# PrimeIntellect-ai/prime

Measured on AMD Instinct MI355X. Metric: tokens_per_sec, higher is better.
Workload: dtype bf16; 1 GPU; model=intellect_10b, global_batch=8, seq_len=2048, parallelism=diloco1_h100_int8ring

## Files before the change

### prime_amd/ops/_lib.py

```python
from __future__ import annotations

import ctypes
from typing import Optional

import torch

from .build import LIB_PATH, build, needs_build

_LIB: Optional[ctypes.CDLL] = None
_TRIED = False

_SIGS = {
    "prime_rmsnorm_fwd": [ctypes.c_void_p] * 5 + [ctypes.c_int64] * 2 + [ctypes.c_double],
    "prime_rmsnorm_bwd": [ctypes.c_void_p] * 7 + [ctypes.c_int64] * 3 + [ctypes.c_double],
    "prime_add_rmsnorm_fwd": [ctypes.c_void_p] * 7 + [ctypes.c_int64] * 2 + [ctypes.c_double],
    "prime_add_rmsnorm_bwd": [ctypes.c_void_p] * 8 + [ctypes.c_int64] * 3 + [ctypes.c_double],
    "prime_rope": [ctypes.c_void_p] * 5 + [ctypes.c_int64] * 4 + [ctypes.c_int, ctypes.c_int64, ctypes.c_void_p],
    "prime_rope_strided": [ctypes.c_void_p] * 5 + [ctypes.c_int64] * 7,
    "prime_qkv_grad_pack": [ctypes.c_void_p] * 8 + [ctypes.c_int64] * 6,
    "prime_swiglu_bwd_t": [ctypes.c_void_p] * 5 + [ctypes.c_int64] * 2,
    "prime_swiglu_fwd": [ctypes.c_void_p] * 3 + [ctypes.c_int64] * 2,
    "prime_swiglu_bwd": [ctypes.c_void_p] * 4 + [ctypes.c_int64] * 2,
    "prime_adamw": [ctypes.c_void_p] * 7 + [ctypes.c_int64] + [ctypes.c_double] * 5 + [ctypes.c_int64],
    "prime_grad_sqnorm": [ctypes.c_void_p] * 3 + [ctypes.c_int64] * 2,
    "prime_grad_sqnorm_partials": [],
    "prime_pseudograd": [ctypes.c_void_p] * 4 + [ctypes.c_int64],
    "prime_quant_int8": [ctypes.c_void_p] * 4 + [ctypes.c_int64],
    "prime_dequant_int8": [ctypes.c_void_p] * 4 + [ctypes.c_int64] * 2,
    "prime_nesterov_outer": [ctypes.c_void_p] * 6 + [ctypes.c_int64] + [ctypes.c_double] * 2,
    "prime_cross_entropy": [ctypes.c_void_p] * 5 + [ctypes.c_int64] * 2 + [ctypes.c_double] + [ctypes.c_int64] * 2,
    "prime_flash_fwd": [ctypes.c_void_p] * 6 + [ctypes.c_int64] * 5 + [ctypes.c_double] + [ctypes.c_int64] * 7 + [ctypes.c_void_p],
    "prime_attn_delta": [ctypes.c_void_p] * 4 + [ctypes.c_int64] * 2,
    "prime_flash_bwd_dq": [ctypes.c_void_p] * 9 + [ctypes.c_int64] * 5 + [ctypes.c_double] + [ctypes.c_int64] * 10 + [ctypes.c_void_p],
    "prime_flash_bwd_dkv": [ctypes.c_void_p] * 13 + [ctypes.c_int64] * 6 + [ctypes.c_double] + [ctypes.c_int64] * 10 + [ctypes.c_void_p],
    "prime_mfma_probe": [ctypes.c_void_p] * 4,
    "prime_mfma_probe32": [ctypes.c_void_p] * 4,
    "prime_transpose_bshd": [ctypes.c_void_p] * 3 + [ctypes.c_int64] * 7,
    "prime_attn_decode": [ctypes.c_void_p] * 5 + [ctypes.c_int64] * 6 + [ctypes.c_double, ctypes.c_void_p],
    "prime_attn_decode_ragged": [ctypes.c_void_p] * 7 + [ctypes.c_int64] * 6 + [ctypes.c_double],
    "prime_decode_ragged_chunk": [],
    "prime_decode_qkv_append": [ctypes.c_void_p] * 8 + [ctypes.c_int64] * 6,
    "prime_gemm_nt": [ctypes.c_void_p] * 4 + [ctypes.c_int64] * 4,
    "prime_gemm_nt8": [ctypes.c_void_p] * 4 + [ctypes.c_int64] * 4,
    "prime_quant_fp8": [ctypes.c_void_p] * 6 + [ctypes.c_int64] * 2,
    "prime_rowwise_quant_fp8": [ctypes.c_void_p] * 4 + [ctypes.c_int64] * 3,
    "prime_transpose_fp8": [ctypes.c_void_p] * 3 + [ctypes.c_int64] * 7 + [ctypes.c_void_p] * 3 + [ctypes.c_int64],
}


def _load() -> ctypes.CDLL:
    import os

    override = os.environ.get("PRIME_AMD_LIB_PATH")
    path = override or str(LIB_PATH)
    if override is None and needs_build():
        build(verbose=True)
    lib = ctypes.CDLL(path)
    for name, argtypes in _SIGS.items():
        try:
            fn = getattr(lib, name)
        except AttributeError:
            continue
        fn.argtypes = argtypes
        fn.restype = ctypes.c_int
    return lib


def lib() -> ctypes.CDLL:
    global _LIB, _TRIED
    if _LIB is None:
        if _TRIED:
            raise RuntimeError("prime_amd HIP kernel library failed to load earlier")
        _TRIED = True
        try:
            _LIB = _load()
        except Exception as e:
            raise RuntimeError(
                "prime_amd requires its HIP kernel library on GPU machines; "
                f"build failed or .so missing at {LIB_PATH}: {e}"
            ) from e
    return _LIB


def have_lib() -> bool:
    try:
        lib()
        return True
    except RuntimeError:
        return False


def stream_of(t: torch.Tensor) -> ctypes.c_void_p:
    s = torch.cuda.current_stream(t.device).cuda_stream
    return ctypes.c_void_p(s)


def check(ret: int, what: str) -> None:
    if ret != 0:
        raise RuntimeError(f"HIP kernel {what} failed with hipError_t={ret}")


def ptr(t: Optional[torch.Tensor]) -> ctypes.c_void_p:
    if t is None:
        return ctypes.c_void_p(0)
    return ctypes.c_void_p(t.data_ptr())
```

### prime_amd/ops/csrc/attention.hip

```cpp
#include "common.h"
#include <stdlib.h>

typedef __attribute__((ext_vector_type(8))) short short8;
typedef __attribute__((ext_vector_type(4))) float f32x4;
typedef __attribute__((address_space(3))) char lds_char;
typedef __attribute__((address_space(3))) void lds_void;
typedef __attribute__((address_space(1))) const void g_void;

__device__ __forceinline__ short8 ld8(const bf16* p) {
  return *reinterpret_cast<const short8*>(p);
}

__device__ __forceinline__ f32x4 mfma16(short8 a, short8 b, f32x4 c) {
  return __builtin_amdgcn_mfma_f32_16x16x32_bf16(a, b, c, 0, 0, 0);
}

__device__ __forceinline__ float grp16_max(float x) {
#pragma unroll
  for (int off = 1; off < 16; off <<= 1) x = fmaxf(x, __shfl_xor(x, off, 64));
  return x;
}
__device__ __forceinline__ float grp16_sum(float x) {
#pragma unroll
  for (int off = 1; off < 16; off <<= 1) x += __shfl_xor(x, off, 64);
// ... 610 lines not shown

  const bf16* Qb = Q + b * sqb + h * sqh;
  const bf16* Kb = K + b * skb + hkv * skh;
  const bf16* Vb = V + b * svb + hkv * svh;
  const bf16* Ktb = Kt + ((int64_t)(b * Hkv + hkv) * D) * S;
  const bf16* dOb = dO + ((int64_t)b * S * H + h) * D;
  const float* lse_b = lse + (int64_t)b * S * H + h;
  const float* dl_b = delta + (int64_t)b * S * H + h;

  __shared__ bf16 k_lds[64 * D];
  __shared__ bf16 v_lds[64 * D];
  __shared__ bf16 kt_lds[D * 64];
  __shared__ bf16 ds_lds_all[4][16 * 64];
  bf16* ds_lds = ds_lds_all[wid];

  short8 qf[DS], dof[DS];
#pragma unroll
  for (int ds = 0; ds < DS; ++ds) {
    qf[ds] = ld8(Qb + (int64_t)(q0 + li) * sqs + ds * 32 + lg * 8);
    dof[ds] = ld8(dOb + (int64_t)(q0 + li) * H * D + ds * 32 + lg * 8);
  }
  float lse_r[4], dl_r[4];
#pragma unroll
  for (int r = 0; r < 4; ++r) {
    lse_r[r] = lse_b[(int64_t)(q0 + lg * 4 + r) * H];
    dl_r[r] = dl_b[(int64_t)(q0 + lg * 4 + r) * H];
  }
  f32x4 dq_acc[DT];
#pragma unroll
  for (int dt = 0; dt < DT; ++dt) dq_acc[dt] = f32x4{0.f, 0.f, 0.f, 0.f};

  const int kv_end = causal ? (qt * 64 + 64) : S;
  int kv_begin = 0, my_kv_begin = 0, row_ds[4];
  if (DOC) {
    const int* doc_b = doc + (int64_t)b * S;
    kv_begin = doc_clamp(doc_b[qt * 64], qt * 64) & ~63;
    my_kv_begin = doc_clamp(doc_b[q0], q0) & ~63;
#pragma unroll
    for (int r = 0; r < 4; ++r) row_ds[r] = doc_b[q0 + lg * 4 + r];
  }
  for (int kv = kv_begin; kv < kv_end; kv += 64) {
    __syncthreads();
    stage_tile<64, D>(Kb + (int64_t)kv * sks, sks, k_lds, threadIdx.x);
    stage_tile<64, D>(Vb + (int64_t)kv * svs, svs, v_lds, threadIdx.x);
    stage_tile<D, 64>(Ktb + kv, S, kt_lds, threadIdx.x);
    __syncthreads();
    if (DOC && kv < my_kv_begin) continue;
#pragma unroll
    for (int sub = 0; sub < 4; ++sub) {
      f32x4 s_acc{0.f, 0.f, 0.f, 0.f}, dp_acc{0.f, 0.f, 0.f, 0.f};
#pragma unroll
      for (int ds = 0; ds < DS; ++ds) {
        s_acc = mfma16(qf[ds], ld8_swz<D>(k_lds, sub * 16 + li, ds * 64 + lg * 16), s_acc);
        dp_acc = mfma16(dof[ds], ld8_swz<D>(v_lds, sub * 16 + li, ds * 64 + lg * 16), dp_acc);
      }
#pragma unroll
      for (int r = 0; r < 4; ++r) {
        const int qg = q0 + lg * 4 + r;
        const int kg = kv + sub * 16 + li;
        float p = __expf(s_acc[r] * scale - lse_r[r]);
        if (causal && kg > qg) p = 0.f;
        if (DOC && kg < row_ds[r]) p = 0.f;
        st16_swz<64>(ds_lds, lg * 4 + r, sub * 16 + li,
                     f2bf(p * (dp_acc[r] - dl_r[r]) * scale));
      }
    }
    wave_lds_fence();
#pragma unroll
    for (int dt = 0; dt < DT; ++dt)
#pragma unroll
      for (int ks = 0; ks < 2; ++ks)
        dq_acc[dt] = mfma16(ld8_swz<64>(ds_lds, li, ks * 64 + lg * 16),
                            ld8_swz<64>(kt_lds, dt * 16 + li, ks * 64 + lg * 16),
                            dq_acc[dt]);
  }
#pragma unroll
  for (int r = 0; r < 4; ++r) {
    bf16* row = dQ + (((int64_t)(b * S + q0 + lg * 4 + r)) * H + h) * D;
#pragma unroll
    for (int dt = 0; dt < DT; ++dt) row[dt * 16 + li] = f2bf(dq_acc[dt][r]);
  }
}

template <int D, int FLAGS>
__global__ __launch_bounds__(512, 2) void flash_bwd_dkv_v5_kernel(
    const bf16* __restrict__ Q, const bf16* __restrict__ Qt,
    const bf16* __restrict__ K, const bf16* __restrict__ V,
    const bf16* __restrict__ dO, const bf16* __restrict__ dOt,
    const float* __restrict__ lse, const float* __restrict__ delta,
    float* __restrict__ wsK, float* __restrict__ wsV, int B, int H, int Hkv,
    int S, float scale, int causal, int splits,
    int64_t sqb, int64_t sqs, int64_t sqh,
    int64_t skb, int64_t sks, int64_t skh,
    int64_t svb, int64_t svs, int64_t svh) {
  constexpr int DSL = D / 16;
  constexpr int DT32 = D / 32;
  const int n_kt = S / 256;
  const int per_split = (B * Hkv) * n_kt;
  const int split = blockIdx.x / per_split;
  const int rem = blockIdx.x - split * per_split;
  const int bh = rem / n_kt;
  const int kt = rem - bh * n_kt;
  const int b = bh / Hkv, hkv = bh - b * Hkv;
  const int group = H / Hkv;
  const int wid = threadIdx.x >> 6;
  const int lane = threadIdx.x & 63;
  const int lo = lane & 31, hi = lane >> 5;
  const int k0w = kt * 256 + wid * 32;

  const bf16* Kb = K + b * skb + hkv * skh;
  const bf16* Vb = V + b * svb + hkv * svh;

  __shared__ bf16 q_lds[2][64 * D];
  __shared__ bf16 do_lds[2][64 * D];
  __shared__ bf16 qt_lds[2][D * 64];
  __shared__ bf16 dot_lds[2][D * 64];

  const bf16* krow = Kb + (int64_t)(k0w + lo) * sks;
  const bf16* vrow = Vb + (int64_t)(k0w + lo) * svs;
  f32x16 dk_acc[DT32], dv_acc[DT32];
#pragma unroll
  for (int dt = 0; dt < DT32; ++dt)
#pragma unroll
    for (int r = 0; r < 16; ++r) { dk_acc[dt][r] = 0.f; dv_acc[dt][r] = 0.f; }

  const int q_start = (causal ? kt * 256 : 0) + split * 64;
  const int tiles_per_g = (S - q_start + 64 * splits - 1) / (64 * splits);
  const int n_iter = group * tiles_per_g;
  const auto stage_for = [&](int it, int buf) {
    const int g = it / tiles_per_g;
    const int q0g = q_start + (it - g * tiles_per_g) * 64 * splits;
    const int h = hkv * group + g;
    const bf16* Qb_ = Q + b * sqb + h * sqh;
    const bf16* dOb_ = dO + ((int64_t)b * S * H + h) * D;
    const bf16* Qtb = Qt + ((int64_t)(b * H + h) * D) * S;
    const bf16* dOtb = dOt + ((int64_t)(b * H + h) * D) * S;
    stage_tile<64, D, 512>(Qb_ + (int64_t)q0g * sqs, sqs, q_lds[buf], threadIdx.x);
    stage_tile<64, D, 512>(dOb_ + (int64_t)q0g * H * D, (int64_t)H * D, do_lds[buf], threadIdx.x);
    stage_tile<D, 64, 512>(Qtb + q0g, S, qt_lds[buf], threadIdx.x);
    stage_tile<D, 64, 512>(dOtb + q0g, S, dot_lds[buf], threadIdx.x);
  };
  stage_for(0, 0);
  for (int it = 0; it < n_iter; ++it) {
    const int cur = it & 1;
    __syncthreads();
    if (it + 1 < n_iter)
      stage_for(it + 1, cur ^ 1);
    const int g = it / tiles_per_g;
    const int q0g = q_start + (it - g * tiles_per_g) * 64 * splits;
    if (causal && q0g + 64 <= k0w) continue;
    const int h = hkv * group + g;
    const float* lse_b = lse + (int64_t)b * S * H + h;
    const float* dl_b = delta + (int64_t)b * S * H + h;

#pragma unroll
    for (int qs = 0; qs < 2; ++qs) {
      const int q32 = q0g + qs * 32;
      f32x16 st, dpt;
#pragma unroll
      for (int r = 0; r < 16; ++r) { st[r] = 0.f; dpt[r] = 0.f; }
      if (FLAGS & 1) __builtin_amdgcn_s_setprio(1);
#pragma unroll
      for (int ds = 0; ds < DSL; ++ds) {
        const short8 qfr = ld8_swz<D>(q_lds[cur], qs * 32 + lo, ds * 32 + hi * 16);
        st = mfma32(qfr, ld8(krow + ds * 16 + hi * 8), st);
      }
#pragma unroll
      for (int ds = 0; ds < DSL; ++ds) {
        const short8 dofr = ld8_swz<D>(do_lds[cur], qs * 32 + lo, ds * 32 + hi * 16);
        dpt = mfma32(dofr, ld8(vrow + ds * 16 + hi * 8), dpt);
      }
      if (FLAGS & 1) __builtin_amdgcn_s_setprio(0);
#pragma unroll
      for (int r = 0; r < 16; ++r) {
        const int qg = q32 + (r & 3) + 8 * (r >> 2) + 4 * hi;
        const float lse_q = lse_b[(int64_t)qg * H];
        const float dl_q = dl_b[(int64_t)qg * H];
        float p = __expf(st[r] * scale - lse_q);
        if (causal && (k0w + lo) > qg) p = 0.f;
        st[r] = p;
        dpt[r] = p * (dpt[r] - dl_q) * scale;
      }
      short8 pa[2], da[2];
#pragma unroll
      for (int kst = 0; kst < 2; ++kst) {
        const int g0 = 4 * (2 * kst), g1 = 4 * (2 * kst + 1);
        unsigned x0 = cvt_pk_bf16(st[g0 + 0], st[g0 + 1]);
        unsigned x1 = cvt_pk_bf16(st[g0 + 2], st[g0 + 3]);
        unsigned y0 = cvt_pk_bf16(st[g1 + 0], st[g1 + 1]);
        unsigned y1 = cvt_pk_bf16(st[g1 + 2], st[g1 + 3]);
        permlane32_swap(x0, y0);
        permlane32_swap(x1, y1);
        short8 f;
        reinterpret_cast<unsigned*>(&f)[0] = x0;
        reinterpret_cast<unsigned*>(&f)[1] = x1;
        reinterpret_cast<unsigned*>(&f)[2] = y0;
        reinterpret_cast<unsigned*>(&f)[3] = y1;
        pa[kst] = f;
        x0 = cvt_pk_bf16(dpt[g0 + 0], dpt[g0 + 1]);
        x1 = cvt_pk_bf16(dpt[g0 + 2], dpt[g0 + 3]);
        y0 = cvt_pk_bf16(dpt[g1 + 0], dpt[g1 + 1]);
        y1 = cvt_pk_bf16(dpt[g1 + 2], dpt[g1 + 3]);
        permlane32_swap(x0, y0);
        permlane32_swap(x1, y1);
        reinterpret_cast<unsigned*>(&f)[0] = x0;
        reinterpret_cast<unsigned*>(&f)[1] = x1;
        reinterpret_cast<unsigned*>(&f)[2] = y0;
        reinterpret_cast<unsigned*>(&f)[3] = y1;
        da[kst] = f;
      }
      if (FLAGS & 1) __builtin_amdgcn_s_setprio(1);
#pragma unroll
      for (int dt = 0; dt < DT32; ++dt)
#pragma unroll
        for (int kst = 0; kst < 2; ++kst) {
          const int colb = qs * 64 + kst * 32 + hi * 16;
          dv_acc[dt] = mfma32(pa[kst],
                              ld8_swz<64>(dot_lds[cur], dt * 32 + lo, colb),
                              dv_acc[dt]);
          dk_acc[dt] = mfma32(da[kst],
                              ld8_swz<64>(qt_lds[cur], dt * 32 + lo, colb),
                              dk_acc[dt]);
        }
      if (FLAGS & 1) __builtin_amdgcn_s_setprio(0);
    }
  }
#pragma unroll
  for (int r = 0; r < 16; ++r) {
    const int kg = k0w + (r & 3) + 8 * (r >> 2) + 4 * hi;
    const int64_t base = ((((int64_t)split * B + b) * Hkv + hkv) * S + kg) * D;
#pragma unroll
    for (int dt = 0; dt < DT32; ++dt) {
      wsK[base + dt * 32 + lo] = dk_acc[dt][r];
      wsV[base + dt * 32 + lo] = dv_acc[dt][r];
    }
  }
}

template <int D, int NW = 4, int DBUF = 1, bool DOC = false>
__global__ __launch_bounds__(512) void flash_bwd_dkv_kernel(
    const bf16* __restrict__ Q, const bf16* __restrict__ Qt,
    const bf16* __restrict__ K, const bf16* __restrict__ V,
    const bf16* __restrict__ dO, const bf16* __restrict__ dOt,
    const float* __restrict__ lse, const float* __restrict__ delta,
    float* __restrict__ wsK, float* __restrict__ wsV, int B, int H, int Hkv,
    int S, float scale, int causal, int splits,
    int64_t sqb, int64_t sqs, int64_t sqh,
    int64_t skb, int64_t sks, int64_t skh,
    int64_t svb, int64_t svs, int64_t svh,
    const int* __restrict__ doc_end) {
  constexpr int DS = D / 32;
  constexpr int DT = D / 16;
  const int n_kt = S / (NW * 16);
  const int per_split = (B * Hkv) * n_kt;
  const int split = blockIdx.x / per_split;
  const int rem = blockIdx.x - split * per_split;
  const int bh = rem / n_kt;
  const int kt = rem - bh * n_kt;
  const int b = bh / Hkv, hkv = bh - b * Hkv;
  const int group = H / Hkv;
  const int wid = threadIdx.x >> 6;
  const int lane = threadIdx.x & 63;
  const int lg = lane >> 4, li = lane & 15;
  const int k0 = kt * (NW * 16) + wid * 16;

  const bf16* Kb = K + b * skb + hkv * skh;
  const bf16* Vb = V + b * svb + hkv * svh;

  __shared__ bf16 q_lds[DBUF][64 * D];
  __shared__ bf16 do_lds[DBUF][64 * D];
  __shared__ bf16 qt_lds[DBUF][D * 64];
  __shared__ bf16 dot_lds[DBUF][D * 64];
  __shared__ bf16 pt_lds_all[NW][16 * 64];
  __shared__ bf16 dst_lds_all[NW][16 * 64];
  bf16* pt_lds = pt_lds_all[wid];
  bf16* dst_lds = dst_lds_all[wid];

  short8 kf[DS], vf[DS];
#pragma unroll
  for (int ds = 0; ds < DS; ++ds) {
    kf[ds] = ld8(Kb + (int64_t)(k0 + li) * sks + ds * 32 + lg * 8);
    vf[ds] = ld8(Vb + (int64_t)(k0 + li) * svs + ds * 32 + lg * 8);
  }
  f32x4 dk_acc[DT], dv_acc[DT];
#pragma unroll
  for (int dt = 0; dt < DT; ++dt) {
    dk_acc[dt] = f32x4{0.f, 0.f, 0.f, 0.f};
    dv_acc[dt] = f32x4{0.f, 0.f, 0.f, 0.f};
  }

  const int q_start = (causal ? (kt * (NW * 16)) / 64 * 64 : 0) + split * 64;
  int q_end = S, my_q_end = S, key_end[4];
  if (DOC) {
    const int* de_b = doc_end + (int64_t)b * S;
    q_end = (doc_clamp(de_b[kt * (NW * 16) + NW * 16 - 1], S) + 63) & ~63;
    my_q_end = doc_clamp(de_b[k0 + 15], S);
#pragma unroll
    for (int r = 0; r < 4; ++r) key_end[r] = de_b[k0 + lg * 4 + r];
  }
  const int tiles_per_g =
      (q_end > q_start) ? (q_end - q_start + 64 * splits - 1) / (64 * splits) : 0;
  const int n_iter = group * tiles_per_g;
  const auto stage_it = [&](int it, int buf) {
    const int g_ = it / tiles_per_g;
    const int q0g_ = q_start + (it - g_ * tiles_per_g) * 64 * splits;
    const int h_ = hkv * group + g_;
    const bf16* Qb_ = Q + b * sqb + h_ * sqh;
    const bf16* dOb_ = dO + ((int64_t)b * S * H + h_) * D;
// ... 182 lines not shown
                     (const int*)nullptr)
  {
    const int grid = (int)(B * H * (S / 64));
    if (D == 128) LAUNCH_FWD(128, 4); else LAUNCH_FWD(64, 4);
  }
  return (int)hipGetLastError();
}

PRIME_API int prime_attn_delta(hipStream_t stream, const void* dO,
                               const void* O, void* delta, int64_t rows,
                               int64_t D) {
  int grid = prime_grid(rows * 64, 256);
  hipLaunchKernelGGL(attn_delta_kernel, dim3(grid), dim3(256), 0, stream,
                     (const bf16*)dO, (const bf16*)O, (float*)delta, rows,
                     (int)D);
  return (int)hipGetLastError();
}

PRIME_API int prime_flash_bwd_dq(hipStream_t stream, const void* Q,
                                 const void* K, const void* V, const void* Kt,
                                 const void* dO, const void* lse,
                                 const void* delta, void* dQ, int64_t B,
                                 int64_t H, int64_t Hkv, int64_t S, int64_t D,
                                 double scale, int64_t causal,
                                 int64_t sqb, int64_t sqs, int64_t sqh,
                                 int64_t skb, int64_t sks, int64_t skh,
                                 int64_t svb, int64_t svs, int64_t svh,
                                 const void* doc_start) {
  if (S % 64 != 0 || (D != 64 && D != 128)) return hipErrorInvalidValue;
  static const char* v5env = getenv("PRIME_ATTN_V5");
  static const char* flagenv = getenv("PRIME_ATTN_FLAGS");
  const int flags = flagenv ? atoi(flagenv) : 2;
  if (doc_start) {
    if (!causal) return hipErrorInvalidValue;
    const bool v5 = (S % 256 == 0) && !(v5env && v5env[0] == '0');
#define LAUNCH_DQ_DOC(KER, QT, NT)                                           \
    hipLaunchKernelGGL(KER, dim3((int)(B * H * (S / QT))), dim3(NT), 0,      \
                       stream, (const bf16*)Q, (const bf16*)K,               \
                       (const bf16*)V, (const bf16*)Kt, (const bf16*)dO,     \
                       (const float*)lse, (const float*)delta, (bf16*)dQ,    \
                       (int)B, (int)H, (int)Hkv, (int)S, (float)scale, 1,    \
                       sqb, sqs, sqh, skb, sks, skh, svb, svs, svh,          \
                       (const int*)doc_start)
    if (v5 && D == 128) LAUNCH_DQ_DOC((flash_bwd_dq_v5_kernel<128, 0, true>), 256, 512);
    else if (v5) LAUNCH_DQ_DOC((flash_bwd_dq_v5_kernel<64, 0, true>), 256, 512);
    else if (D == 128) LAUNCH_DQ_DOC((flash_bwd_dq_kernel<128, true>), 64, 256);
    else LAUNCH_DQ_DOC((flash_bwd_dq_kernel<64, true>), 64, 256);
    return (int)hipGetLastError();
  }
  if ((D == 64) && (S % 256 == 0) && !(v5env && v5env[0] == '0')) {
    const int grid = (int)(B * H * (S / 256));
    hipLaunchKernelGGL((flash_bwd_dq_v5_kernel<64, 0>), dim3(grid),
                       dim3(512), 0, stream, (const bf16*)Q, (const bf16*)K,
                       (const bf16*)V, (const bf16*)Kt, (const bf16*)dO,
                       (const float*)lse, (const float*)delta, (bf16*)dQ,
                       (int)B, (int)H, (int)Hkv, (int)S, (float)scale,
                       (int)causal, sqb, sqs, sqh, skb, sks, skh,
                       svb, svs, svh, (const int*)nullptr);
    return (int)hipGetLastError();
  }
  if ((D == 128) && (S % 256 == 0) && !(v5env && v5env[0] == '0')) {
    const int grid = (int)(B * H * (S / 256));
#define LAUNCH_DQ5(F)                                                       \
    hipLaunchKernelGGL((flash_bwd_dq_v5_kernel<128, F>), dim3(grid),        \
                       dim3(512), 0, stream, (const bf16*)Q,                \
                       (const bf16*)K, (const bf16*)V, (const bf16*)Kt,     \
                       (const bf16*)dO, (const float*)lse,                  \
                       (const float*)delta, (bf16*)dQ, (int)B, (int)H,      \
                       (int)Hkv, (int)S, (float)scale, (int)causal,         \
                       sqb, sqs, sqh, skb, sks, skh, svb, svs, svh,         \
                       (const int*)nullptr)
    if (flags & 1) LAUNCH_DQ5(1); else LAUNCH_DQ5(0);
    return (int)hipGetLastError();
  }
  const int grid = (int)(B * H * (S / 64));
  DISPATCH_D(flash_bwd_dq_kernel, (const bf16*)Q, (const bf16*)K,
             (const bf16*)V, (const bf16*)Kt, (const bf16*)dO,
             (const float*)lse, (const float*)delta, (bf16*)dQ, (int)B, (int)H,
             (int)Hkv, (int)S, (float)scale, (int)causal, sqb, sqs, sqh, skb,
             sks, skh, svb, svs, svh, (const int*)nullptr);
  return (int)hipGetLastError();
}

PRIME_API int prime_flash_bwd_dkv(hipStream_t stream, const void* Q,
                                  const void* Qt, const void* K, const void* V,
                                  const void* dO, const void* dOt,
                                  const void* lse, const void* delta, void* dK,
                                  void* dV, void* wsK, void* wsV,
                                  int64_t splits, int64_t B, int64_t H,
                                  int64_t Hkv, int64_t S, int64_t D,
                                  double scale, int64_t causal,
                                  int64_t sqb, int64_t sqs, int64_t sqh,
                                  int64_t skb, int64_t sks, int64_t skh,
                                  int64_t svb, int64_t svs, int64_t svh,
                                  const void* doc_end) {
  if (S % 64 != 0 || (D != 64 && D != 128)) return hipErrorInvalidValue;
  if (doc_end && !causal) return hipErrorInvalidValue;
  static const char* v5denv = getenv("PRIME_ATTN_DKV5");
  static const char* fenv = getenv("PRIME_ATTN_FLAGS");
  const int flags = fenv ? atoi(fenv) : 2;
  if (!doc_end && (D == 128) && (S % 256 == 0) && (v5denv && v5denv[0] == '1')) {
    const int sp = (int)(splits > 4 ? 4 : splits);
    const int grid = (int)(B * Hkv * (S / 256) * sp);
#define LAUNCH_DKV5(F)                                                       \
    hipLaunchKernelGGL((flash_bwd_dkv_v5_kernel<128, F>), dim3(grid),        \
                       dim3(512), 0, stream, (const bf16*)Q,                 \
                       (const bf16*)Qt, (const bf16*)K, (const bf16*)V,      \
                       (const bf16*)dO, (const bf16*)dOt,                    \
                       (const float*)lse, (const float*)delta, (float*)wsK,  \
                       (float*)wsV, (int)B, (int)H, (int)Hkv, (int)S,        \
                       (float)scale, (int)causal, sp, sqb, sqs, sqh,         \
                       skb, sks, skh, svb, svs, svh)
    if (flags & 1) LAUNCH_DKV5(1); else LAUNCH_DKV5(0);
    int err5 = hipGetLastError();
    if (err5) return err5;
    int rgrid5 = prime_grid(B * Hkv * S * D, 256);
    hipLaunchKernelGGL(dkv_reduce_kernel, dim3(rgrid5), dim3(256), 0, stream,
                       (const float*)wsK, (const float*)wsV, (bf16*)dK,
                       (bf16*)dV, (int)B, (int)Hkv, (int)S, (int)D, sp);
    return (int)hipGetLastError();
  }
  static const char* nw8env = getenv("PRIME_ATTN_DKV8");
  const bool nw8 = (S % 128 == 0) && !(nw8env && nw8env[0] == '0');
#define LAUNCH_DKV(DD, NWV, DB) LAUNCH_DKV_(DD, NWV, DB, false, nullptr)
#define LAUNCH_DKV_DOC(DD, NWV, DB) LAUNCH_DKV_(DD, NWV, DB, true, doc_end)
#define LAUNCH_DKV_(DD, NWV, DB, DOCV, DOCP)                                 \
    hipLaunchKernelGGL((flash_bwd_dkv_kernel<DD, NWV, DB, DOCV>),            \
                       dim3((int)(B * Hkv * (S / (NWV * 16)) * splits)),     \
                       dim3(NWV * 64), 0, stream, (const bf16*)Q,            \
                       (const bf16*)Qt, (const bf16*)K, (const bf16*)V,      \
                       (const bf16*)dO, (const bf16*)dOt,                    \
                       (const float*)lse, (const float*)delta, (float*)wsK,  \
                       (float*)wsV, (int)B, (int)H, (int)Hkv, (int)S,        \
                       (float)scale, (int)causal, (int)splits, sqb, sqs,     \
                       sqh, skb, sks, skh, svb, svs, svh, (const int*)DOCP)
  static const char* dbenv = getenv("PRIME_ATTN_DKV_DBUF");
  const bool dbuf = !(dbenv && dbenv[0] == '0');
  if (doc_end) {
    if (nw8 && dbuf) {
      if (D == 128) LAUNCH_DKV_DOC(128, 8, 2); else LAUNCH_DKV_DOC(64, 8, 2);
    } else if (nw8) {
      if (D == 128) LAUNCH_DKV_DOC(128, 8, 1); else LAUNCH_DKV_DOC(64, 8, 1);
    } else {
      if (D == 128) LAUNCH_DKV_DOC(128, 4, 1); else LAUNCH_DKV_DOC(64, 4, 1);
    }
  } else if (nw8 && dbuf) {
    if (D == 128) LAUNCH_DKV(128, 8, 2); else LAUNCH_DKV(64, 8, 2);
  } else if (nw8) {
    if (D == 128) LAUNCH_DKV(128, 8, 1); else LAUNCH_DKV(64, 8, 1);
  } else {
    if (D == 128) LAUNCH_DKV(128, 4, 1); else LAUNCH_DKV(64, 4, 1);
  }
  int err = hipGetLastError();
  if (err) return err;
  int rgrid = prime_grid(B * Hkv * S * D, 256);
  hipLaunchKernelGGL(dkv_reduce_kernel, dim3(rgrid), dim3(256), 0, stream,
                     (const float*)wsK, (const float*)wsV, (bf16*)dK,
                     (bf16*)dV, (int)B, (int)Hkv, (int)S, (int)D, (int)splits);
  return (int)hipGetLastError();
}
```

### prime_amd/ops/functional.py

```python
from __future__ import annotations

import torch

from . import reference as ref
from ._lib import check, lib, ptr, stream_of

_DW_ROWS = 1024


def _is_hip(t: torch.Tensor) -> bool:
    return t.is_cuda


class _RMSNorm(torch.autograd.Function):
    @staticmethod
    def forward(ctx, x: torch.Tensor, w: torch.Tensor, eps: float):
        if not _is_hip(x):
            ctx.save_for_backward(x, w)
            ctx.eps = eps
            return ref.rmsnorm(x, w, eps)
        x = x.contiguous()
        shp = x.shape
        D = shp[-1]
        if D % 8 != 0:
# ... 196 lines not shown
            f"swiglu kernel needs intermediate dim % 8 == 0 (got {I})")
    check(lib().prime_swiglu_bwd(stream_of(gu), ptr(dout), ptr(gu), ptr(dgu), R, I),
          "swiglu_bwd")
    return dgu, dgu.view(R, 2 * I).t().contiguous()


def transpose_bshd(x: torch.Tensor) -> torch.Tensor:
    B, S, H, D = x.shape
    if not x.is_cuda or S % 64 != 0 or D % 64 != 0 or x.stride(3) != 1:
        return x.permute(0, 2, 3, 1).contiguous()
    out = torch.empty(B, H, D, S, device=x.device, dtype=x.dtype)
    check(
        lib().prime_transpose_bshd(
            stream_of(x), ptr(x), ptr(out), B, S, H, D,
            x.stride(0), x.stride(1), x.stride(2),
        ),
        "transpose_bshd",
    )
    return out


def _bshd_ok(t: torch.Tensor) -> bool:
    sb, ss, sh, sd = t.stride()
    return sd == 1 and sb % 8 == 0 and ss % 8 == 0 and sh % 8 == 0 \
        and t.storage_offset() % 8 == 0


def _check_flash_shape(S: int, D: int) -> None:
    if D not in (64, 128) or S % 64 != 0:
        raise NotImplementedError(
            f"flash attention kernels support head_dim in {{64, 128}} and "
            f"seq_len % 64 == 0 (got head_dim={D}, seq_len={S}); pad the "
            "sequence or pick a head_dim-compatible model config"
        )


def doc_starts(tokens: torch.Tensor, eos_id: int) -> torch.Tensor:
    B, S = tokens.shape
    idx = torch.arange(S, device=tokens.device, dtype=torch.int32).expand(B, S)
    new_doc = torch.zeros(B, S, dtype=torch.bool, device=tokens.device)
    new_doc[:, 1:] = tokens[:, :-1] == eos_id
    return torch.where(new_doc, idx, torch.zeros_like(idx)).cummax(dim=1).values


def _doc_ends(doc_start: torch.Tensor) -> torch.Tensor:
    B, S = doc_start.shape
    idx = torch.arange(S, device=doc_start.device, dtype=torch.int32).expand(B, S)
    cand = torch.where(doc_start == idx, idx, torch.full_like(idx, S))
    nxt = cand.flip(1).cummin(dim=1).values.flip(1)
    return torch.cat([nxt[:, 1:], torch.full_like(idx[:, :1], S)], dim=1).contiguous()


_DOC_END_CACHE: list = [None, None, None]


def _doc_ends_cached(doc_start: torch.Tensor) -> torch.Tensor:
    import weakref

    ref_, ver, val = _DOC_END_CACHE
    if ref_ is not None and ref_() is doc_start and ver == doc_start._version:
        return val
    val = _doc_ends(doc_start)
    _DOC_END_CACHE[:] = [weakref.ref(doc_start), doc_start._version, val]
    return val


def _check_doc_start(doc_start, q, causal: bool) -> None:
    B, S = q.shape[0], q.shape[1]
    if not causal:
        raise ValueError("flash_attention: doc_start requires causal=True")
    if not isinstance(doc_start, torch.Tensor) or doc_start.dtype != torch.int32:
        raise TypeError(
            "flash_attention: doc_start must be an int32 tensor "
            f"(got {getattr(doc_start, 'dtype', type(doc_start))})")
    if tuple(doc_start.shape) != (B, S):
        raise ValueError(
            f"flash_attention: doc_start must have shape [B, S] = [{B}, {S}] "
            f"(got {list(doc_start.shape)})")
    if doc_start.device != q.device:
        raise ValueError(
            f"flash_attention: doc_start is on {doc_start.device}, q on {q.device}")


class _FlashAttention(torch.autograd.Function):

    @staticmethod
    def forward(ctx, q, k, v, causal: bool, scale: float, doc_start=None):
        B, S, H, D = q.shape
        _check_flash_shape(S, D)
        Hkv = k.shape[2]
        if not (_bshd_ok(q) and _bshd_ok(k) and _bshd_ok(v)):
            q, k, v = q.contiguous(), k.contiguous(), v.contiguous()
        if doc_start is not None:
            doc_start = doc_start.contiguous()
        vt = transpose_bshd(v)
        o = torch.empty(B, S, H, D, device=q.device, dtype=q.dtype)
        lse = torch.empty(B, S, H, device=q.device, dtype=torch.float32)
        check(
            lib().prime_flash_fwd(
                stream_of(q), ptr(q), ptr(k), ptr(vt), ptr(o), ptr(lse),
                B, H, Hkv, S, D, scale, int(causal),
                q.stride(0), q.stride(1), q.stride(2),
                k.stride(0), k.stride(1), k.stride(2), ptr(doc_start),
            ),
            "flash_fwd",
        )
        ctx.save_for_backward(q, k, v, o, lse)
        ctx.meta = (causal, scale)
        ctx.doc_start = doc_start
        return o

    @staticmethod
    def backward(ctx, do):
        q, k, v, o, lse = ctx.saved_tensors
        causal, scale = ctx.meta
        doc_start = ctx.doc_start
        doc_end = _doc_ends_cached(doc_start) if doc_start is not None else None
        B, S, H, D = q.shape
        Hkv = k.shape[2]
        do = do.contiguous()
        delta = torch.empty(B * S * H, device=q.device, dtype=torch.float32)
        check(
            lib().prime_attn_delta(stream_of(q), ptr(do), ptr(o), ptr(delta), B * S * H, D),
            "attn_delta",
        )
        kt = transpose_bshd(k)
        dq = torch.empty(B, S, H, D, device=q.device, dtype=q.dtype)
        check(
            lib().prime_flash_bwd_dq(
                stream_of(q), ptr(q), ptr(k), ptr(v), ptr(kt), ptr(do),
                ptr(lse), ptr(delta), ptr(dq), B, H, Hkv, S, D, scale,
                int(causal),
                q.stride(0), q.stride(1), q.stride(2),
                k.stride(0), k.stride(1), k.stride(2),
                v.stride(0), v.stride(1), v.stride(2), ptr(doc_start),
            ),
            "flash_bwd_dq",
        )
        qt = transpose_bshd(q)
        dot = transpose_bshd(do)
        dk = torch.empty(B, S, Hkv, D, device=q.device, dtype=q.dtype)
        dv = torch.empty(B, S, Hkv, D, device=q.device, dtype=q.dtype)
        import os

        env = os.environ.get("PRIME_AMD_DKV_SPLITS")
        if env:
            splits = max(1, min(int(env), S // 64))
        else:
            splits = max(1, min(8, S // 1024, S // 64))
        ws = torch.empty(2, splits, B, Hkv, S, D, device=q.device,
                         dtype=torch.float32)
        check(
            lib().prime_flash_bwd_dkv(
                stream_of(q), ptr(q), ptr(qt), ptr(k), ptr(v), ptr(do),
                ptr(dot), ptr(lse), ptr(delta), ptr(dk), ptr(dv),
                ptr(ws[0]), ptr(ws[1]), splits,
                B, H, Hkv, S, D, scale, int(causal),
                q.stride(0), q.stride(1), q.stride(2),
                k.stride(0), k.stride(1), k.stride(2),
                v.stride(0), v.stride(1), v.stride(2), ptr(doc_end),
            ),
            "flash_bwd_dkv",
        )
        return dq, dk, dv, None, None, None


def flash_attention(q, k, v, causal: bool = True, doc_start=None) -> torch.Tensor:
    if doc_start is not None:
        _check_doc_start(doc_start, q, causal)
    if not _is_hip(q):
        return ref.attention(q, k, v, causal, doc_start=doc_start)
    if doc_start is None:
        return _FlashAttention.apply(q, k, v, causal, q.shape[-1] ** -0.5)
    return _FlashAttention.apply(q, k, v, causal, q.shape[-1] ** -0.5, doc_start)


class _CrossEntropy(torch.autograd.Function):
    @staticmethod
    def forward(ctx, logits, targets, ignore_index: int, need_grad: bool):
        R, V = logits.shape
        logits = logits.contiguous()
        t32 = targets.to(torch.int32).contiguous()
        loss = torch.empty(R, device=logits.device, dtype=torch.float32)
        dlogits = torch.empty_like(logits) if need_grad else logits
        check(
            lib().prime_cross_entropy(
                stream_of(logits), ptr(logits), ptr(t32), ptr(loss), ptr(dlogits),
                R, V, 1.0, ignore_index, 1 if need_grad else 0,
            ),
            "cross_entropy",
        )
        n_valid = (targets != ignore_index).sum().clamp(min=1)
        if need_grad:
            ctx.save_for_backward(dlogits, n_valid)
        else:
            ctx.save_for_backward(torch.empty(0, device=logits.device,
                                              dtype=logits.dtype), n_valid)
        return loss.sum() / n_valid.float()

    @staticmethod
    def backward(ctx, grad_out):
        dlogits, n_valid = ctx.saved_tensors
        g = dlogits * (grad_out.float() / n_valid.float()).to(dlogits.dtype)
        return g, None, None, None


def cross_entropy(logits, targets, ignore_index: int = -100) -> torch.Tensor:
    if not _is_hip(logits):
        return ref.cross_entropy(logits, targets, ignore_index)
    need_grad = torch.is_grad_enabled() and logits.requires_grad
    return _CrossEntropy.apply(logits, targets, ignore_index, need_grad)


_WT_EPOCH = 0
_WT_CACHE: dict = {}
_LINEAR_TUNED = False


def set_linear_tuned(on: bool) -> None:
    global _LINEAR_TUNED
    _LINEAR_TUNED = bool(on)
    _WT_CACHE.clear()


def invalidate_wt_cache() -> None:
    global _WT_EPOCH
    _WT_EPOCH += 1
    _WT_CACHE.clear()
    _FP8_CACHE.clear()


def _wt_of(w: torch.Tensor):
    N, K = w.shape
    if K % 128 or N % 64:
        return None
    key = (w.data_ptr(), N, K)
    hit = _WT_CACHE.get(key)
    if hit is not None and hit[0] == _WT_EPOCH:
        return hit[1]
    wt = transpose_bshd(w.view(1, N, K // 128, 128)).view(K, N)
    _WT_CACHE[key] = (_WT_EPOCH, wt)
    return wt

# ... 604 lines not shown
```

Measured before the change: 16520 tokens/s.

## Enable reworked 32x32 MFMA dK/dV backward kernel by default for long sequences

Rewrites the previously opt-in v5 dK/dV flash-backward kernel as a 256-thread, 128-key-tile kernel. K and V are held in registers, and lse/delta rows are prefetched into LDS alongside the double-buffered Q/dO stages. It adds explicit sched_group_barrier interleaving of MFMA, LDS reads and VALU softmax, plus doc-mask support. Auto mode now selects it when D==128 and S>=2048. The aim is better MFMA utilisation and fewer scattered global loads in attention backward, at the cost of higher register pressure and hand-tuned scheduling that may not suit the compiler.

```diff
diff --git a/prime_amd/ops/_lib.py b/prime_amd/ops/_lib.py
--- a/prime_amd/ops/_lib.py
+++ b/prime_amd/ops/_lib.py
@@ -32,7 +32,8 @@
     "prime_flash_fwd": [ctypes.c_void_p] * 6 + [ctypes.c_int64] * 5 + [ctypes.c_double] + [ctypes.c_int64] * 7 + [ctypes.c_void_p],
     "prime_attn_delta": [ctypes.c_void_p] * 4 + [ctypes.c_int64] * 2,
     "prime_flash_bwd_dq": [ctypes.c_void_p] * 9 + [ctypes.c_int64] * 5 + [ctypes.c_double] + [ctypes.c_int64] * 10 + [ctypes.c_void_p],
-    "prime_flash_bwd_dkv": [ctypes.c_void_p] * 13 + [ctypes.c_int64] * 6 + [ctypes.c_double] + [ctypes.c_int64] * 10 + [ctypes.c_void_p],
+    "prime_flash_bwd_dkv": [ctypes.c_void_p] * 13 + [ctypes.c_int64] * 6 + [ctypes.c_double] + [ctypes.c_int64] * 10 + [ctypes.c_void_p, ctypes.c_int64],
+    "prime_flash_bwd_dkv_kernel_for": [ctypes.c_int64] * 3,
     "prime_mfma_probe": [ctypes.c_void_p] * 4,
     "prime_mfma_probe32": [ctypes.c_void_p] * 4,
     "prime_transpose_bshd": [ctypes.c_void_p] * 3 + [ctypes.c_int64] * 7,
diff --git a/prime_amd/ops/csrc/attention.hip b/prime_amd/ops/csrc/attention.hip
--- a/prime_amd/ops/csrc/attention.hip
+++ b/prime_amd/ops/csrc/attention.hip
@@ -716,8 +716,11 @@
   }
 }
 
-template <int D, int FLAGS>
-__global__ __launch_bounds__(512, 2) void flash_bwd_dkv_v5_kernel(
+#ifndef PRIME_DKV32_NV
+#define PRIME_DKV32_NV 9
+#endif
+template <int D, bool DOC = false>
+__global__ __launch_bounds__(256) void flash_bwd_dkv_v5_kernel(
     const bf16* __restrict__ Q, const bf16* __restrict__ Qt,
     const bf16* __restrict__ K, const bf16* __restrict__ V,
     const bf16* __restrict__ dO, const bf16* __restrict__ dOt,
@@ -726,10 +729,12 @@
     int S, float scale, int causal, int splits,
     int64_t sqb, int64_t sqs, int64_t sqh,
     int64_t skb, int64_t sks, int64_t skh,
-    int64_t svb, int64_t svs, int64_t svh) {
+    int64_t svb, int64_t svs, int64_t svh,
+    const int* __restrict__ doc_end) {
   constexpr int DSL = D / 16;
   constexpr int DT32 = D / 32;
-  const int n_kt = S / 256;
+  constexpr int KT = 128;
+  const int n_kt = S / KT;
   const int per_split = (B * Hkv) * n_kt;
   const int split = blockIdx.x / per_split;
   const int rem = blockIdx.x - split * per_split;
@@ -740,7 +745,7 @@
   const int wid = threadIdx.x >> 6;
   const int lane = threadIdx.x & 63;
   const int lo = lane & 31, hi = lane >> 5;
-  const int k0w = kt * 256 + wid * 32;
+  const int k0w = kt * KT + wid * 32;
 
   const bf16* Kb = K + b * skb + hkv * skh;
   const bf16* Vb = V + b * svb + hkv * svh;
@@ -749,115 +754,191 @@
   __shared__ bf16 do_lds[2][64 * D];
   __shared__ bf16 qt_lds[2][D * 64];
   __shared__ bf16 dot_lds[2][D * 64];
-
-  const bf16* krow = Kb + (int64_t)(k0w + lo) * sks;
-  const bf16* vrow = Vb + (int64_t)(k0w + lo) * svs;
+  __shared__ __attribute__((aligned(16))) float rc_lds[2][2][64];
+
+  short8 kreg[DSL], vreg[DSL];
+  {
+    const bf16* krow = Kb + (int64_t)(k0w + lo) * sks + hi * 8;
+    const bf16* vrow = Vb + (int64_t)(k0w + lo) * svs + hi * 8;
+#pragma unroll
+    for (int ds = 0; ds < DSL; ++ds) {
+      kreg[ds] = ld8(krow + ds * 16);
+      vreg[ds] = ld8(vrow + ds * 16);
+    }
+  }
   f32x16 dk_acc[DT32], dv_acc[DT32];
 #pragma unroll
   for (int dt = 0; dt < DT32; ++dt)
 #pragma unroll
     for (int r = 0; r < 16; ++r) { dk_acc[dt][r] = 0.f; dv_acc[dt][r] = 0.f; }
 
-  const int q_start = (causal ? kt * 256 : 0) + split * 64;
-  const int tiles_per_g = (S - q_start + 64 * splits - 1) / (64 * splits);
+  const int q_start = (causal ? kt * KT : 0) + split * 64;
+  int q_end = S, my_q_end = S, key_end = S;
+  if (DOC) {
+    const int* de_b = doc_end + (int64_t)b * S;
+    q_end = (doc_clamp(de_b[kt * KT + KT - 1], S) + 63) & ~63;
+    my_q_end = doc_clamp(de_b[k0w + 31], S);
+    key_end = de_b[k0w + lo];
+  }
+  const int tiles_per_g =
+      (q_end > q_start) ? (q_end - q_start + 64 * splits - 1) / (64 * splits) : 0;
   const int n_iter = group * tiles_per_g;
-  const auto stage_for = [&](int it, int buf) {
-    const int g = it / tiles_per_g;
-    const int q0g = q_start + (it - g * tiles_per_g) * 64 * splits;
-    const int h = hkv * group + g;
-    const bf16* Qb_ = Q + b * sqb + h * sqh;
-    const bf16* dOb_ = dO + ((int64_t)b * S * H + h) * D;
-    const bf16* Qtb = Qt + ((int64_t)(b * H + h) * D) * S;
-    const bf16* dOtb = dOt + ((int64_t)(b * H + h) * D) * S;
-    stage_tile<64, D, 512>(Qb_ + (int64_t)q0g * sqs, sqs, q_lds[buf], threadIdx.x);
-    stage_tile<64, D, 512>(dOb_ + (int64_t)q0g * H * D, (int64_t)H * D, do_lds[buf], threadIdx.x);
-    stage_tile<D, 64, 512>(Qtb + q0g, S, qt_lds[buf], threadIdx.x);
-    stage_tile<D, 64, 512>(dOtb + q0g, S, dot_lds[buf], threadIdx.x);
+  const auto stage_it = [&](int it, int buf) {
+    const int g_ = it / tiles_per_g;
+    const int q0g_ = q_start + (it - g_ * tiles_per_g) * 64 * splits;
+    const int h_ = hkv * group + g_;
+    const bf16* Qb_ = Q + b * sqb + h_ * sqh;
+    const bf16* dOb_ = dO + ((int64_t)b * S * H + h_) * D;
+    const bf16* Qtb_ = Qt + ((int64_t)(b * H + h_) * D) * S;
+    const bf16* dOtb_ = dOt + ((int64_t)(b * H + h_) * D) * S;
+    stage_tile<64, D, 256>(Qb_ + (int64_t)q0g_ * sqs, sqs, q_lds[buf], threadIdx.x);
+    stage_tile<64, D, 256>(dOb_ + (int64_t)q0g_ * H * D, (int64_t)H * D, do_lds[buf], threadIdx.x);
+    stage_tile<D, 64, 256>(Qtb_ + q0g_, S, qt_lds[buf], threadIdx.x);
+    stage_tile<D, 64, 256>(dOtb_ + q0g_, S, dot_lds[buf], threadIdx.x);
   };
-  stage_for(0, 0);
+  const auto load_rc = [&](int it) -> float {
+    if (wid >= 2) return 0.f;
+    const int g_ = it / tiles_per_g;
+    const int q0g_ = q_start + (it - g_ * tiles_per_g) * 64 * splits;
+    const int h_ = hkv * group + g_;
+    const float* src = (wid == 0 ? lse : delta) + (int64_t)b * S * H + h_;
+    return src[(int64_t)(q0g_ + lane) * H];
+  };
+  const auto store_rc = [&](int buf, float x) {
+    if (wid < 2) rc_lds[buf][wid][lane] = x;
+  };
+  if (n_iter > 0) {
+    const float rc0 = load_rc(0);
+    stage_it(0, 0);
+    store_rc(0, rc0);
+  }
   for (int it = 0; it < n_iter; ++it) {
     const int cur = it & 1;
     __syncthreads();
-    if (it + 1 < n_iter)
-      stage_for(it + 1, cur ^ 1);
+#pragma unroll
+    for (int dt = 0; dt < DT32; ++dt)
+      asm volatile("" : "+a"(dk_acc[dt]), "+a"(dv_acc[dt]));
+    const bool more = it + 1 < n_iter;
+    float rc_next = 0.f;
+    if (more) {
+      rc_next = load_rc(it + 1);
+      stage_it(it + 1, cur ^ 1);
+    }
     const int g = it / tiles_per_g;
     const int q0g = q_start + (it - g * tiles_per_g) * 64 * splits;
-    if (causal && q0g + 64 <= k0w) continue;
-    const int h = hkv * group + g;
-    const float* lse_b = lse + (int64_t)b * S * H + h;
-    const float* dl_b = delta + (int64_t)b * S * H + h;
-
-#pragma unroll
-    for (int qs = 0; qs < 2; ++qs) {
-      const int q32 = q0g + qs * 32;
-      f32x16 st, dpt;
-#pragma unroll
-      for (int r = 0; r < 16; ++r) { st[r] = 0.f; dpt[r] = 0.f; }
-      if (FLAGS & 1) __builtin_amdgcn_s_setprio(1);
-#pragma unroll
-      for (int ds = 0; ds < DSL; ++ds) {
-        const short8 qfr = ld8_swz<D>(q_lds[cur], qs * 32 + lo, ds * 32 + hi * 16);
-        st = mfma32(qfr, ld8(krow + ds * 16 + hi * 8), st);
-      }
-#pragma unroll
-      for (int ds = 0; ds < DSL; ++ds) {
-        const short8 dofr = ld8_swz<D>(do_lds[cur], qs * 32 + lo, ds * 32 + hi * 16);
-        dpt = mfma32(dofr, ld8(vrow + ds * 16 + hi * 8), dpt);
-      }
-      if (FLAGS & 1) __builtin_amdgcn_s_setprio(0);
-#pragma unroll
-      for (int r = 0; r < 16; ++r) {
-        const int qg = q32 + (r & 3) + 8 * (r >> 2) + 4 * hi;
-        const float lse_q = lse_b[(int64_t)qg * H];
-        const float dl_q = dl_b[(int64_t)qg * H];
-        float p = __expf(st[r] * scale - lse_q);
-        if (causal && (k0w + lo) > qg) p = 0.f;
-        st[r] = p;
-        dpt[r] = p * (dpt[r] - dl_q) * scale;
-      }
-      short8 pa[2], da[2];
-#pragma unroll
-      for (int kst = 0; kst < 2; ++kst) {
-        const int g0 = 4 * (2 * kst), g1 = 4 * (2 * kst + 1);
-        unsigned x0 = cvt_pk_bf16(st[g0 + 0], st[g0 + 1]);
-        unsigned x1 = cvt_pk_bf16(st[g0 + 2], st[g0 + 3]);
-        unsigned y0 = cvt_pk_bf16(st[g1 + 0], st[g1 + 1]);
-        unsigned y1 = cvt_pk_bf16(st[g1 + 2], st[g1 + 3]);
-        permlane32_swap(x0, y0);
-        permlane32_swap(x1, y1);
-        short8 f;
-        reinterpret_cast<unsigned*>(&f)[0] = x0;
-        reinterpret_cast<unsigned*>(&f)[1] = x1;
-        reinterpret_cast<unsigned*>(&f)[2] = y0;
-        reinterpret_cast<unsigned*>(&f)[3] = y1;
-        pa[kst] = f;
-        x0 = cvt_pk_bf16(dpt[g0 + 0], dpt[g0 + 1]);
-        x1 = cvt_pk_bf16(dpt[g0 + 2], dpt[g0 + 3]);
-        y0 = cvt_pk_bf16(dpt[g1 + 0], dpt[g1 + 1]);
-        y1 = cvt_pk_bf16(dpt[g1 + 2], dpt[g1 + 3]);
-        permlane32_swap(x0, y0);
-        permlane32_swap(x1, y1);
-        reinterpret_cast<unsigned*>(&f)[0] = x0;
-        reinterpret_cast<unsigned*>(&f)[1] = x1;
-        reinterpret_cast<unsigned*>(&f)[2] = y0;
-        reinterpret_cast<unsigned*>(&f)[3] = y1;
-        da[kst] = f;
-      }
-      if (FLAGS & 1) __builtin_amdgcn_s_setprio(1);
-#pragma unroll
-      for (int dt = 0; dt < DT32; ++dt)
+    const bool skip = (causal && q0g + 64 <= k0w) || (DOC && q0g >= my_q_end);
+    if (!skip) {
+      f32x16 st[2], dpt[2];
+      short8 pa[2][2], da[2][2];
+      short8 fs[2][2 * DSL], fa[2][4 * DT32];
+#pragma unroll
+      for (int qs = 0; qs < 2; ++qs)
+#pragma unroll
+        for (int r = 0; r < 16; ++r) { st[qs][r] = 0.f; dpt[qs][r] = 0.f; }
+      const auto load_s = [&](int qs) {
+#pragma unroll
+        for (int ds = 0; ds < DSL; ++ds) {
+          fs[qs][ds] = ld8_swz<D>(q_lds[cur], qs * 32 + lo, ds * 32 + hi * 16);
+          fs[qs][DSL + ds] = ld8_swz<D>(do_lds[cur], qs * 32 + lo, ds * 32 + hi * 16);
+        }
+      };
+      const auto mfma_s = [&](int qs) {
+#pragma unroll
+        for (int ds = 0; ds < DSL; ++ds) {
+          st[qs] = mfma32(fs[qs][ds], kreg[ds], st[qs]);
+          dpt[qs] = mfma32(fs[qs][DSL + ds], vreg[ds], dpt[qs]);
+        }
+      };
+      const auto load_acc = [&](int qs) {
+#pragma unroll
+        for (int dt = 0; dt < DT32; ++dt)
+#pragma unroll
+          for (int kst = 0; kst < 2; ++kst) {
+            const int colb = qs * 64 + kst * 32 + hi * 16;
+            fa[qs][(dt * 2 + kst) * 2] = ld8_swz<64>(dot_lds[cur], dt * 32 + lo, colb);
+            fa[qs][(dt * 2 + kst) * 2 + 1] = ld8_swz<64>(qt_lds[cur], dt * 32 + lo, colb);
+          }
+      };
+      const auto mfma_acc = [&](int qs) {
+#pragma unroll
+        for (int dt = 0; dt < DT32; ++dt)
+#pragma unroll
+          for (int kst = 0; kst < 2; ++kst) {
+            dv_acc[dt] = mfma32(pa[qs][kst], fa[qs][(dt * 2 + kst) * 2], dv_acc[dt]);
+            dk_acc[dt] = mfma32(da[qs][kst], fa[qs][(dt * 2 + kst) * 2 + 1], dk_acc[dt]);
+          }
+      };
+      const auto softmax = [&](int qs) {
+#pragma unroll
+        for (int r4 = 0; r4 < 4; ++r4) {
+          const int row = qs * 32 + 8 * r4 + 4 * hi;
+          const f32x4 lse4 = *reinterpret_cast<const f32x4*>(&rc_lds[cur][0][row]);
+          const f32x4 dl4 = *reinterpret_cast<const f32x4*>(&rc_lds[cur][1][row]);
+#pragma unroll
+          for (int j = 0; j < 4; ++j) {
+            const int r = 4 * r4 + j;
+            const int qg = q0g + row + j;
+            float p = __expf(st[qs][r] * scale - lse4[j]);
+            if (causal && (k0w + lo) > qg) p = 0.f;
+            if (DOC && qg >= key_end) p = 0.f;
+            st[qs][r] = p;
+            dpt[qs][r] = p * (dpt[qs][r] - dl4[j]) * scale;
+          }
+        }
 #pragma unroll
         for (int kst = 0; kst < 2; ++kst) {
-          const int colb = qs * 64 + kst * 32 + hi * 16;
-          dv_acc[dt] = mfma32(pa[kst],
-                              ld8_swz<64>(dot_lds[cur], dt * 32 + lo, colb),
-                              dv_acc[dt]);
-          dk_acc[dt] = mfma32(da[kst],
-                              ld8_swz<64>(qt_lds[cur], dt * 32 + lo, colb),
-                              dk_acc[dt]);
+          const int g0 = 4 * (2 * kst), g1 = 4 * (2 * kst + 1);
+          unsigned x0 = cvt_pk_bf16(st[qs][g0 + 0], st[qs][g0 + 1]);
+          unsigned x1 = cvt_pk_bf16(st[qs][g0 + 2], st[qs][g0 + 3]);
+          unsigned y0 = cvt_pk_bf16(st[qs][g1 + 0], st[qs][g1 + 1]);
+          unsigned y1 = cvt_pk_bf16(st[qs][g1 + 2], st[qs][g1 + 3]);
+          permlane32_swap(x0, y0);
+          permlane32_swap(x1, y1);
+          short8 f;
+          reinterpret_cast<unsigned*>(&f)[0] = x0;
+          reinterpret_cast<unsigned*>(&f)[1] = x1;
+          reinterpret_cast<unsigned*>(&f)[2] = y0;
+          reinterpret_cast<unsigned*>(&f)[3] = y1;
+          pa[qs][kst] = f;
+          x0 = cvt_pk_bf16(dpt[qs][g0 + 0], dpt[qs][g0 + 1]);
+          x1 = cvt_pk_bf16(dpt[qs][g0 + 2], dpt[qs][g0 + 3]);
+          y0 = cvt_pk_bf16(dpt[qs][g1 + 0], dpt[qs][g1 + 1]);
+          y1 = cvt_pk_bf16(dpt[qs][g1 + 2], dpt[qs][g1 + 3]);
+          permlane32_swap(x0, y0);
+          permlane32_swap(x1, y1);
+          reinterpret_cast<unsigned*>(&f)[0] = x0;
+          reinterpret_cast<unsigned*>(&f)[1] = x1;
+          reinterpret_cast<unsigned*>(&f)[2] = y0;
+          reinterpret_cast<unsigned*>(&f)[3] = y1;
+          da[qs][kst] = f;
         }
-      if (FLAGS & 1) __builtin_amdgcn_s_setprio(0);
-    }
+      };
+#define DKV32_PATTERN(NV)                                        \
+      _Pragma("unroll") for (int i_ = 0; i_ < 16; ++i_) {        \
+        __builtin_amdgcn_sched_group_barrier(0x008, 1, 0);       \
+        __builtin_amdgcn_sched_group_barrier(0x100, 1, 0);       \
+        if (NV) __builtin_amdgcn_sched_group_barrier(0x002, NV, 0); \
+      }
+      load_s(0);
+      __builtin_amdgcn_sched_barrier(0);
+      load_s(1);
+      mfma_s(0);
+      DKV32_PATTERN(0)
+      __builtin_amdgcn_sched_barrier(0);
+      load_acc(0);
+      mfma_s(1);
+      softmax(0);
+      DKV32_PATTERN(PRIME_DKV32_NV)
+      __builtin_amdgcn_sched_barrier(0);
+      load_acc(1);
+      mfma_acc(0);
+      softmax(1);
+      DKV32_PATTERN(PRIME_DKV32_NV)
+      __builtin_amdgcn_sched_barrier(0);
+      mfma_acc(1);
+#undef DKV32_PATTERN
+    }
+    if (more) store_rc(cur ^ 1, rc_next);
   }
 #pragma unroll
   for (int r = 0; r < 16; ++r) {
@@ -1206,6 +1287,15 @@
   return (int)hipGetLastError();
 }
 
+PRIME_API int prime_flash_bwd_dkv_kernel_for(int64_t S, int64_t D,
+                                             int64_t variant) {
+  const bool ok32 = (D == 128) && (S % 128 == 0);
+  if (variant == 1) return 1;
+  if (variant == 2) return ok32 ? 2 : -1;
+  if (variant != 0) return -1;
+  return (ok32 && S >= 2048) ? 2 : 1;
+}
+
 PRIME_API int prime_flash_bwd_dkv(hipStream_t stream, const void* Q,
                                   const void* Qt, const void* K, const void* V,
                                   const void* dO, const void* dOt,
@@ -1217,31 +1307,31 @@
                                   int64_t sqb, int64_t sqs, int64_t sqh,
                                   int64_t skb, int64_t sks, int64_t skh,
                                   int64_t svb, int64_t svs, int64_t svh,
-                                  const void* doc_end) {
+                                  const void* doc_end, int64_t variant) {
   if (S % 64 != 0 || (D != 64 && D != 128)) return hipErrorInvalidValue;
   if (doc_end && !causal) return hipErrorInvalidValue;
-  static const char* v5denv = getenv("PRIME_ATTN_DKV5");
-  static const char* fenv = getenv("PRIME_ATTN_FLAGS");
-  const int flags = fenv ? atoi(fenv) : 2;
-  if (!doc_end && (D == 128) && (S % 256 == 0) && (v5denv && v5denv[0] == '1')) {
-    const int sp = (int)(splits > 4 ? 4 : splits);
-    const int grid = (int)(B * Hkv * (S / 256) * sp);
-#define LAUNCH_DKV5(F)                                                       \
-    hipLaunchKernelGGL((flash_bwd_dkv_v5_kernel<128, F>), dim3(grid),        \
-                       dim3(512), 0, stream, (const bf16*)Q,                 \
-                       (const bf16*)Qt, (const bf16*)K, (const bf16*)V,      \
-                       (const bf16*)dO, (const bf16*)dOt,                    \
-                       (const float*)lse, (const float*)delta, (float*)wsK,  \
-                       (float*)wsV, (int)B, (int)H, (int)Hkv, (int)S,        \
-                       (float)scale, (int)causal, sp, sqb, sqs, sqh,         \
-                       skb, sks, skh, svb, svs, svh)
-    if (flags & 1) LAUNCH_DKV5(1); else LAUNCH_DKV5(0);
-    int err5 = hipGetLastError();
-    if (err5) return err5;
-    int rgrid5 = prime_grid(B * Hkv * S * D, 256);
-    hipLaunchKernelGGL(dkv_reduce_kernel, dim3(rgrid5), dim3(256), 0, stream,
+  if (splits < 1) return hipErrorInvalidValue;
+  const int which = prime_flash_bwd_dkv_kernel_for(S, D, variant);
+  if (which < 0) return hipErrorInvalidValue;
+  if (which == 2) {
+#define LAUNCH_DKV32(DOCV, DOCP)                                             \
+    hipLaunchKernelGGL((flash_bwd_dkv_v5_kernel<128, DOCV>),                 \
+                       dim3((int)(B * Hkv * (S / 128) * splits)), dim3(256), \
+                       0, stream, (const bf16*)Q, (const bf16*)Qt,           \
+                       (const bf16*)K, (const bf16*)V, (const bf16*)dO,      \
+                       (const bf16*)dOt, (const float*)lse,                  \
+                       (const float*)delta, (float*)wsK, (float*)wsV,        \
+                       (int)B, (int)H, (int)Hkv, (int)S, (float)scale,       \
+                       (int)causal, (int)splits, sqb, sqs, sqh, skb, sks,    \
+                       skh, svb, svs, svh, (const int*)DOCP)
+    if (doc_end) LAUNCH_DKV32(true, doc_end); else LAUNCH_DKV32(false, nullptr);
+    int err32 = hipGetLastError();
+    if (err32) return err32;
+    int rgrid32 = prime_grid(B * Hkv * S * D, 256);
+    hipLaunchKernelGGL(dkv_reduce_kernel, dim3(rgrid32), dim3(256), 0, stream,
                        (const float*)wsK, (const float*)wsV, (bf16*)dK,
-                       (bf16*)dV, (int)B, (int)Hkv, (int)S, (int)D, sp);
+                       (bf16*)dV, (int)B, (int)Hkv, (int)S, (int)D,
+                       (int)splits);
     return (int)hipGetLastError();
   }
   static const char* nw8env = getenv("PRIME_ATTN_DKV8");
diff --git a/prime_amd/ops/functional.py b/prime_amd/ops/functional.py
--- a/prime_amd/ops/functional.py
+++ b/prime_amd/ops/functional.py
@@ -302,6 +302,9 @@
             f"flash_attention: doc_start is on {doc_start.device}, q on {q.device}")
 
 
+_DKV_VARIANTS = {"auto": 0, "16": 1, "32": 2}
+
+
 class _FlashAttention(torch.autograd.Function):
 
     @staticmethod
@@ -363,6 +366,16 @@
         dv = torch.empty(B, S, Hkv, D, device=q.device, dtype=q.dtype)
         import os
 
+        mode = os.environ.get("PRIME_AMD_DKV_KERNEL") or "auto"
+        if mode not in _DKV_VARIANTS:
+            raise ValueError(
+                f"PRIME_AMD_DKV_KERNEL must be one of {sorted(_DKV_VARIANTS)} (got {mode!r})")
+        variant = _DKV_VARIANTS[mode]
+        kernel = lib().prime_flash_bwd_dkv_kernel_for(S, D, variant)
+        if kernel < 0:
+            raise ValueError(
+                f"PRIME_AMD_DKV_KERNEL={mode}: the 32x32 dK/dV kernel needs D == 128 "
+                f"and S % 128 == 0 (got S={S}, D={D})")
         env = os.environ.get("PRIME_AMD_DKV_SPLITS")
         if env:
             splits = max(1, min(int(env), S // 64))
@@ -378,7 +391,7 @@
                 B, H, Hkv, S, D, scale, int(causal),
                 q.stride(0), q.stride(1), q.stride(2),
                 k.stride(0), k.stride(1), k.stride(2),
-                v.stride(0), v.stride(1), v.stride(2), ptr(doc_end),
+                v.stride(0), v.stride(1), v.stride(2), ptr(doc_end), variant,
             ),
             "flash_bwd_dkv",
         )
```

Result: no change. 16520 tokens/s (median of 3 runs) (+0.0%).
